# rusty-fast-solvers/rusty-compression

Hardware: AMD Instinct MI355X
Metric: GB/s + compressions/sec, 8192x8192 f64 rank-128 rSVD+ID (higher is better)
Workload: dtype f64

## Files before the change

### rusty_compression_amd/csrc/kernels_qr.hip

```cpp
#include "rc_common.hpp"
#include "rc_device.hpp"

namespace rc {

static __host__ __device__ inline int64_t cdiv(int64_t a, int64_t b) { return (a + b - 1) / b; }

template <typename T> struct Num;
template <> struct Num<double> {
    static __host__ __device__ inline double tol3z() { return 1.0536712127723509e-08; }
};
template <> struct Num<float> {
    static __host__ __device__ inline float tol3z() { return 2.44140625e-04f; }
};

template <typename T>
__device__ inline T wsum(T v) {
#pragma unroll
    for (int off = 32; off > 0; off >>= 1) v += __shfl_xor(v, off, 64);
    return v;
}

template <typename T, int TPC>
__device__ inline T group_sum(T v, T *sh ) {
    v = wsum(v);
    if (TPC == 256) {
        __syncthreads();
        if ((threadIdx.x & 63) == 0) sh[threadIdx.x >> 6] = v;
        __syncthreads();
        v = sh[0] + sh[1] + sh[2] + sh[3];
    }
    return v;
}

template <typename T>
// ... 239 lines not shown
    const int64_t m = w.rows, n = w.cols;
    if (m == 0 || n == 0) return;
    kmax = std::min(kmax, std::min(m, n));
    ProfScope ps(c, "op:geqp3 %lldx%lld k=%lld pivot=%d", (long long)m, (long long)n, (long long)kmax, pivot ? 1 : 0);
    T *vn1 = vn, *vn2 = vn + n;
    const int pv = pivot ? 1 : 0;
    hipLaunchKernelGGL(k_qr_init<T>, dim3((unsigned)std::min<int64_t>(n, 65535)), dim3(256), 0, c->stream, w, pv, jpvt, vn1, vn2);
    for (int64_t j = 0; j < kmax; ++j) {
        hipLaunchKernelGGL(k_qr_pivot_reflect<T>, dim3(1), dim3(1024), 0, c->stream, w, j, pv, jpvt, vn1, vn2, tau);
        const int64_t rem_cols = n - j - 1;
        if (rem_cols <= 0) continue;
        const int64_t rem = m - j;
        const int64_t c64 = cdiv(rem, 64), c256 = cdiv(rem, 256);
#define RC_APPLY(TPC, MAXE)                                                                                       \
    hipLaunchKernelGGL((k_qr_apply<T, TPC, MAXE>), dim3((unsigned)cdiv(rem_cols, 256 / TPC)), dim3(256), 0,      \
                       c->stream, w, j, pv, jpvt, vn1, vn2, tau)
        if (c64 <= 2 && rem_cols >= 2048) {
            constexpr int CPW = 4;
            hipLaunchKernelGGL((k_qr_apply_short<T, CPW>), dim3((unsigned)cdiv(rem_cols, 4 * CPW)), dim3(256), 0, c->stream, w, j, pv, jpvt, vn1, vn2, tau);
        }
        else if (c64 <= 2) RC_APPLY(64, 2);
        else if (c64 <= 8) RC_APPLY(64, 8);
        else if (c256 <= 8) RC_APPLY(256, 8);
        else if (c256 <= 16) RC_APPLY(256, 16);
        else if (c256 <= 32) RC_APPLY(256, 32);
        else
            hipLaunchKernelGGL(k_qr_apply_general<T>, dim3((unsigned)rem_cols), dim3(256), 0, c->stream, w, j, pv, jpvt, vn1, vn2, tau);
#undef RC_APPLY
    }
}

template <typename T>
__global__ __launch_bounds__(256) void k_extract_r(Mat<T> w, const int64_t *jpvt, Mat<T> r) {
    const bool col_fast = (r.cs <= r.rs);
    const int64_t total = r.rows * r.cols;
    for (int64_t e = blockIdx.x * (int64_t)blockDim.x + threadIdx.x; e < total; e += (int64_t)gridDim.x * blockDim.x) {
        int64_t i, p;
        if (col_fast) { i = e / r.cols; p = e - i * r.cols; }
        else { p = e / r.rows; i = e - p * r.rows; }
        r.at(i, p) = (i <= p) ? w.p[jpvt[p] * w.cs + i] : (T)0;
    }
}
template <typename T>
void extract_r(rc_context *c, Mat<T> w, const int64_t *jpvt, Mat<T> r) {
    if (r.empty()) return;
    int grid = (int)std::min<int64_t>(cdiv(r.rows * r.cols, 256), 8192);
    hipLaunchKernelGGL(k_extract_r<T>, dim3(grid), dim3(256), 0, c->stream, w, jpvt, r);
}

template <typename T, int MAXE>
__global__ __launch_bounds__(256) void k_form_q(Mat<T> w, const int64_t *jpvt, const T *tau, int64_t k, Mat<T> qw) {
    __shared__ T sh[4];
    const int64_t m = w.rows;
    const int64_t cq = blockIdx.x;
    const int tid = threadIdx.x;
    T x[MAXE];
#pragma unroll
    for (int e = 0; e < MAXE; ++e) {
        int64_t i = tid + (int64_t)e * 256;
        x[e] = (i == cq) ? (T)1 : (T)0;
    }
    for (int64_t j = (cq < k - 1 ? cq : k - 1); j >= 0; --j) {
        const T tj = tau[j];
        if (tj == (T)0) continue;
        const T *vcol = w.p + jpvt[j] * w.cs;
        T v[MAXE];
        T dot = 0;
#pragma unroll
        for (int e = 0; e < MAXE; ++e) {
            const int i = tid + e * 256;
            const bool ok = i < (int)m && i >= (int)j;
            const T vv = vcol[ok ? i : (int)j];
            v[e] = ok ? (i == (int)j ? (T)1 : vv) : (T)0;
            dot = fma(v[e], x[e], dot);
// ... 5 lines not shown
    }
    T *out = qw.p + cq * qw.cs;
#pragma unroll
    for (int e = 0; e < MAXE; ++e) {
        int64_t i = tid + (int64_t)e * 256;
        if (i < m) out[i] = x[e];
    }
}
template <typename T>
__global__ __launch_bounds__(256) void k_form_q_general(Mat<T> w, const int64_t *jpvt, const T *tau, int64_t k, Mat<T> qw) {
    __shared__ T sh[4];
    const int64_t m = w.rows;
    const int64_t cq = blockIdx.x;
    const int tid = threadIdx.x;
    T *x = qw.p + cq * qw.cs;
    for (int64_t i = tid; i < m; i += 256) x[i] = (i == cq) ? (T)1 : (T)0;
    for (int64_t j = (cq < k - 1 ? cq : k - 1); j >= 0; --j) {
        const T tj = tau[j];
        if (tj == (T)0) continue;
        const T *vcol = w.p + jpvt[j] * w.cs;
        const int64_t i0 = tid >= j ? tid : tid + ((j - tid + 255) / 256) * 256;
        T dot = 0;
        for (int64_t i = i0; i < m; i += 256) dot += ((i == j) ? (T)1 : vcol[i]) * x[i];
        dot = group_sum<T, 256>(dot, sh);
        const T f = tj * dot;
        for (int64_t i = i0; i < m; i += 256) x[i] -= f * ((i == j) ? (T)1 : vcol[i]);
    }
}

template <typename T, int NE>
__global__ __launch_bounds__(1024) void k_form_q_small(Mat<T> w, const int64_t *jpvt, const T *tau, int k, Mat<T> qw) {
    extern __shared__ __attribute__((aligned(16))) char smem_raw[];
    T *V = reinterpret_cast<T *>(smem_raw);
    T *tl = V + (size_t)k * 8 * NE;
    const int m = (int)w.rows;
    constexpr int LD = 8 * NE;
    for (int e = threadIdx.x; e < k * LD; e += blockDim.x) {
        const int j = e / LD, i = e - j * LD;
        V[e] = (i < j || i >= m) ? (T)0 : (i == j) ? (T)1 : w.p[jpvt[j] * w.cs + i];
    }
    for (int j = threadIdx.x; j < k; j += blockDim.x) tl[j] = tau[j];
    __syncthreads();
    const int l8 = threadIdx.x & 7, cq = threadIdx.x >> 3;
    if (cq >= qw.cols) return;
    T x[NE];
#pragma unroll
    for (int e = 0; e < NE; ++e) x[e] = (l8 + 8 * e == cq) ? (T)1 : (T)0;
    for (int j = cq < k - 1 ? cq : k - 1; j >= 0; --j) {
        const T tj = tl[j];
        if (tj == (T)0) continue;
        const T *vj = V + (size_t)j * LD + l8;
        T v[NE];
        T dot = 0;
#pragma unroll
        for (int e = 0; e < NE; ++e) {
            v[e] = vj[8 * e];
            dot = fma(v[e], x[e], dot);
        }
        dot = group_sum_dpp<8>(dot);
        const T f = tj * dot;
#pragma unroll
        for (int e = 0; e < NE; ++e) x[e] = fma(-f, v[e], x[e]);
    }
    T *out = qw.p + (int64_t)cq * qw.cs;
#pragma unroll
    for (int e = 0; e < NE; ++e) {
        const int i = l8 + 8 * e;
        if (i < m) out[i] = x[e];
    }
}

template <typename T>
__global__ __launch_bounds__(256) void k_extract_v(Mat<T> w, const int64_t *jpvt, Mat<T> vm) {
    const int64_t j = blockIdx.y;
    const T *col = w.p + jpvt[j] * w.cs;
    T *out = vm.p + j * vm.cs;
    for (int64_t i = blockIdx.x * 256 + threadIdx.x; i < vm.rows; i += (int64_t)gridDim.x * 256)
        out[i] = (i < j) ? (T)0 : (i == j) ? (T)1 : col[i];
}
template <typename T>
__global__ __launch_bounds__(1024) void k_build_t(Mat<T> sgram, const T *tau, Mat<T> tm) {
    extern __shared__ __attribute__((aligned(16))) char smem_raw[];
    T *svec = reinterpret_cast<T *>(smem_raw);
    T *trow = svec + tm.rows;
    const int k = (int)tm.rows;
    const int ld = k | 1;
    const int tid = threadIdx.x;
    for (int e = tid; e < k * ld; e += 1024) trow[e] = 0;
    __syncthreads();
    for (int j = 0; j < k; ++j) {
        for (int l = tid; l < j; l += 1024) svec[l] = sgram.at(l, j);
        __syncthreads();
        const T tj = tau[j];
        for (int i = tid; i <= j; i += 1024) {
            if (i == j) {
                trow[i * ld + j] = tj;
            } else {
                T acc = 0;
                for (int l = i; l < j; ++l) acc += trow[i * ld + l] * svec[l];
                trow[i * ld + j] = -tj * acc;
            }
        }
// ... 463 lines not shown
```

### rusty_compression_amd/csrc/kernels_wqcoop.hip

```cpp
#include "rc_common.hpp"
#include <cstdlib>
#include "rc_device.hpp"
#include "jacobi_lds.hpp"

#include <chrono>
#include <mutex>

#include <cerrno>
#include <csignal>
#include <fcntl.h>
#include <sys/file.h>
#include <sys/mman.h>
#include <unistd.h>

namespace rc {

namespace {

constexpr int kCoopMaxWgs = 128;
constexpr int kSpinLimit = 1 << 22;

template <typename T> struct Tol3z;
template <> struct Tol3z<double> { static __device__ inline double v() { return 1.0536712127723509e-08; } };
template <> struct Tol3z<float> { static __device__ inline float v() { return 2.44140625e-04f; } };

__device__ inline void st_agent(double *p, double v) { __hip_atomic_store(p, v, __ATOMIC_RELAXED, RC_AGENT); }
__device__ inline void st_agent(float *p, float v) { __hip_atomic_store(p, v, __ATOMIC_RELAXED, RC_AGENT); }
__device__ inline void st_agent(long long *p, long long v) { __hip_atomic_store(p, v, __ATOMIC_RELAXED, RC_AGENT); }
__device__ inline void st_agent(unsigned *p, unsigned v) { __hip_atomic_store(p, v, __ATOMIC_RELAXED, RC_AGENT); }
__device__ inline double ld_agent(const double *p) { return __hip_atomic_load(p, __ATOMIC_RELAXED, RC_AGENT); }
__device__ inline float ld_agent(const float *p) { return __hip_atomic_load(p, __ATOMIC_RELAXED, RC_AGENT); }
__device__ inline long long ld_agent(const long long *p) { return __hip_atomic_load(p, __ATOMIC_RELAXED, RC_AGENT); }
__device__ inline unsigned ld_agent(const unsigned *p) { return __hip_atomic_load(p, __ATOMIC_RELAXED, RC_AGENT); }

__global__ void k_coop_gate(unsigned *sem, unsigned need, unsigned budget, unsigned *sync, unsigned long long *hdr, int hdr_words, const int *proceed) {
    if (blockIdx.x != 0) return;
// ... 11 lines not shown
    }
    st_agent(sync + 1, ab);
}

}

#ifdef RC_COOP_TIMING
__device__ unsigned long long g_coop_dbg[8];
#endif

template <typename T>
struct WqCoopArgs {
    Mat<T> w;
    Mat<T> wf;
    int kmax;
    int cpw;
    int64_t *jpvt;
    T *tau;
    unsigned long long *hdr;
    T *cols;
    int mp;
    unsigned *sync;
    unsigned *sem;
    int *flag;
    int row0;
    int jend;
    const int *pos_in;
    int *pos_out;
    T *vn;
    unsigned units;
};

template <typename T, int NE, int CPG>
__device__ inline void wq_coop_body(const WqCoopArgs<T> &a, const int G, const int wg) {
    constexpr int NG = 64;
    constexpr int NW = 8;
    constexpr int kNoInt = 0x7fffffff;
    __shared__ double sh_v[NW];
    __shared__ int sh_p[NW], sh_c[NW], sh_j[NW];
    __shared__ int sh_exit;
    __shared__ int bc[4];
    __shared__ T xw[8 * NE];
    const int tid = threadIdx.x, lane = tid & 63, wv = tid >> 6, l8 = tid & 7, g8 = tid >> 3;
    const int m = (int)a.w.rows, mp = a.mp;
    const int64_t n = a.w.cols;
    const int c0 = wg * a.cpw;
    const int nloc = (int)((n - c0) < a.cpw ? (n - c0) : a.cpw);
    unsigned *done = a.sync, *abortw = a.sync + 1;

    const int row0 = a.row0;
    const unsigned ab0 = ld_agent(abortw);
    if (ab0 == 2u) {
        if (tid == 0 && wg == 0) atomicOr(a.flag, 4);
        return;
    }
    const bool dead = a.pos_in != nullptr && (__hip_atomic_load(a.flag, __ATOMIC_RELAXED, RC_AGENT) & 4) != 0;
    if (tid == 0) sh_exit = (ab0 != 0u) || dead;

    T x[CPG][NE];
    int pos[CPG];
    T myvn1 = 0, myvn2 = 0;
    const int mycol = c0 + g8 + NG * l8;
    const bool resumed = a.pos_in != nullptr;
    const Mat<T> src = resumed ? a.wf : a.w;
#pragma unroll
    for (int q = 0; q < CPG; ++q) {
        const int cl = g8 + NG * q;
        const bool valid = cl < nloc;
        const T *col = src.p + (int64_t)(c0 + (valid ? cl : 0)) * src.cs;
        const int64_t srs = src.rs;
        T ss = 0;
#pragma unroll
        for (int e = 0; e < NE; ++e) {
            const int i = row0 + l8 + 8 * e;
            x[q][e] = (valid && i < m) ? col[(int64_t)i * srs] : (T)0;
            ss = fma(x[q][e], x[q][e], ss);
        }
        ss = group_sum_dpp<8>(ss);
        if (l8 == q && !resumed) myvn1 = myvn2 = sqrt(ss);
        pos[q] = valid ? (resumed ? a.pos_in[c0 + cl] : c0 + cl) : -1;
    }
    if (resumed && l8 < CPG && g8 + NG * l8 < nloc) {
        myvn1 = a.vn[mycol];
        myvn2 = a.vn[n + mycol];
    }
    __syncthreads();
    bool aborted = sh_exit != 0;
// ... 220 lines not shown
    }
    rdone = r0 + 8;
    }
#undef RC_TICK
#ifdef RC_COOP_TIMING
    if (wg == 0 && tid == 0)
        for (int k2 = 0; k2 < 6; ++k2) g_coop_dbg[k2] = tph[k2];
#endif

    if (!aborted) {
#pragma unroll
        for (int q = 0; q < CPG; ++q) {
            if (pos[q] < 0) continue;
            T *col = a.wf.p + (int64_t)(c0 + g8 + NG * q) * a.wf.cs;
#pragma unroll
            for (int e = 0; e < NE; ++e) {
                const int i = rdone + l8 + 8 * e;
                if (i < m) col[i] = x[q][e];
            }
            if (l8 == 0) a.jpvt[pos[q]] = c0 + g8 + NG * q;
            if (l8 == 0 && a.pos_out) a.pos_out[c0 + g8 + NG * q] = pos[q];
        }
        if (a.pos_out && l8 < CPG && g8 + NG * l8 < nloc) {
            a.vn[mycol] = myvn1;
            a.vn[n + mycol] = myvn2;
        }
    }
    __syncthreads();
    if (tid == 0) {
        if (aborted && !dead) atomicOr(a.flag, 4);
        const unsigned old = __hip_atomic_fetch_add(done, 1u, __ATOMIC_ACQ_REL, RC_AGENT);
        if (old == (unsigned)G - 1u) __hip_atomic_fetch_sub(a.sem, a.units, __ATOMIC_RELAXED, RC_AGENT);
    }
}

template <typename T, int NE, int CPG>
__global__ __launch_bounds__(512, NE <= 4 ? 4 : 2) void k_wq_coop(WqCoopArgs<T> a) {
    wq_coop_body<T, NE, CPG>(a, (int)gridDim.x, (int)blockIdx.x);
}

template <typename T>
__global__ __launch_bounds__(512, 2) void k_wq_jacobi_fused(WqCoopArgs<T> a, JacobiLdsArgs<T> ja, int g) {
    const int wg = (int)blockIdx.x;
    if (wg < g) wq_coop_body<T, 16, 4>(a, g, wg);
    else jacobi_lds_body<T, 8, true, 2>(ja, wg == g + 1);
}

static unsigned *coop_semaphore(int device) {
    static std::mutex mu;
    static unsigned *sems[64] = {};
    std::lock_guard<std::mutex> lk(mu);
    unsigned *&s = sems[device & 63];
    if (!s) {
        RC_HIP(hipMalloc(reinterpret_cast<void **>(&s), 64));
        const unsigned zeros[16] = {};
        RC_HIP(hipMemcpy(s, zeros, 64, hipMemcpyHostToDevice));
    }
    return s;
}
void coop_prepare(int device) { (void)coop_semaphore(device); }
unsigned *coop_semaphore_of(int device) { return coop_semaphore(device); }

namespace {
struct ShareTable {
    uint32_t magic;
    uint32_t reserved;
    int32_t pids[62];
};
constexpr uint32_t kShareMagic = 0x52434350u;

struct DeviceShare {
    ShareTable *tab = nullptr;
    int fd = -1;
    bool tried = false;
    int live = 1;
    std::chrono::steady_clock::time_point stamp{};
};

// ... 129 lines not shown
        ProfScope ps(c, "op:geqp3_wide_coop %lldx%lld steps %lld..%lld wgs=%d", (long long)m, (long long)n, (long long)row0, (long long)jend, g);
        if (!last || !first) {
            if (!pos) {
                pos = c->alloc<int>((size_t)n);
                vn = c->alloc<T>((size_t)2 * n);
            }
        }
        WqCoopArgs<T> a = stage_args<T>(c, w, wf, kmax, jpvt, tau, flag, ne, g, cpw);
        a.row0 = (int)row0;
        a.jend = (int)jend;
        a.pos_in = first ? nullptr : pos;
        a.pos_out = last ? nullptr : pos;
        a.vn = vn;
        coop_gate_launch(c, a.units, a.sync, a.hdr, 2 * g * 5);
#define RC_COOP(NE_, CPG_) hipLaunchKernelGGL((k_wq_coop<T, NE_, CPG_>), dim3((unsigned)g), dim3(512), 0, c->stream, a)
        if (ne == 4) RC_COOP(4, 8);
        else if (ne == 8) RC_COOP(8, 8);
        else if (ne == 16) RC_COOP(16, 4);
        else RC_COOP(32, 2);
#undef RC_COOP
        row0 = jend;
        first = false;
    }
}

template <typename T>
bool wide_coop_jacobi_supported(int64_t m, int64_t n, int device) {
    if (!std::is_same<T, double>::value) return false;
    return m == 8 * kLPP && stage_ne(m) == 16 && wide_coop_supported<T>(m, n, device) &&
           jacobi_lds_bytes<T>((int)m, jacobi_pitch<T>((int)m)) <= kJacobiLdsCap;
}

template <typename T>
void geqp3_wide_coop_jacobi(rc_context *c, Mat<T> w, Mat<T> wf, int64_t kmax, int64_t *jpvt, T *tau, int *flag, Mat<T> core, Mat<T> uc, T *s, Mat<T> vc) {
    const int64_t m = w.rows, n = w.cols;
    RC_REQUIRE(wf.rs == 1 && wf.rows == m && wf.cols == n, RC_LAYOUT_ERROR, "geqp3_wide_coop_jacobi: column-major output required");
    RC_REQUIRE(core.rows == m && core.cols == m && core.rs == 1 && uc.rs == 1 && vc.rs == 1, RC_LAYOUT_ERROR, "geqp3_wide_coop_jacobi: square column-major core required");
    RC_REQUIRE(wide_coop_jacobi_supported<T>(m, n, c->device), RC_INVALID_ARGUMENT, "geqp3_wide_coop_jacobi: unsupported shape");
    if constexpr (std::is_same<T, double>::value) {
        kmax = std::min(kmax, std::min(m, n));
        const int nc = (int)m, N = nc;
        int cpg, cpw, g;
        stage_shape(16, n, &cpg, &cpw, &g);
        ProfScope ps(c, "op:geqp3_wide_coop %lldx%lld + jacobi_svd n=%d wgs=%d+2", (long long)m, (long long)n, nc, g);
        const WqCoopArgs<T> a = stage_args<T>(c, w, wf, kmax, jpvt, tau, flag, 16, g, cpw);
        const int ld = jacobi_pitch<T>(nc);
        const size_t lds = jacobi_lds_bytes<T>(nc, ld);
        const size_t nrec = (size_t)kMaxSweeps * (N - 1) * (N / 2);
        Rot<T> *log = c->alloc<Rot<T>>(nrec);
        int *sweeps = c->alloc<int>(1);
        int *order = c->alloc<int>((size_t)nc);
        unsigned *vsync = c->alloc<unsigned>((size_t)nc + 1);
        unsigned long long *chk = c->alloc<unsigned long long>(nrec);
        const JacobiLdsArgs<T> ja{core, log, sweeps, uc, s, order, kMaxSweeps, 1, vsync, chk, c->epoch_word(), vc, c->health_word(), ld};
        auto kern = k_wq_jacobi_fused<T>;
        static bool attr_set[64] = {};
        if (!attr_set[c->device & 63]) {
            RC_HIP(hipFuncSetAttribute(reinterpret_cast<const void *>(kern), hipFuncAttributeMaxDynamicSharedMemorySize, 160 * 1024 - 2048));
            attr_set[c->device & 63] = true;
        }
        fill_words(c, vsync, ((size_t)nc + 1) * sizeof(unsigned), 0u);
        coop_gate_launch(c, a.units, a.sync, a.hdr, 2 * g * 5);
        hipLaunchKernelGGL(kern, dim3((unsigned)g + 2), dim3(512), lds, c->stream, a, ja, g);
    }
}

#ifdef RC_COOP_TIMING
extern "C" void rc_debug_coop_timing(unsigned long long *out) { (void)hipMemcpyFromSymbol(out, HIP_SYMBOL(g_coop_dbg), 8 * sizeof(unsigned long long)); }
#endif
template bool wide_coop_supported<double>(int64_t, int64_t, int);
template bool wide_coop_supported<float>(int64_t, int64_t, int);
template void geqp3_wide_coop<double>(rc_context *, Mat<double>, Mat<double>, int64_t, int64_t *, double *, int *);
template void geqp3_wide_coop<float>(rc_context *, Mat<float>, Mat<float>, int64_t, int64_t *, float *, int *);
template bool wide_coop_jacobi_supported<double>(int64_t, int64_t, int);
template bool wide_coop_jacobi_supported<float>(int64_t, int64_t, int);
template void geqp3_wide_coop_jacobi<double>(rc_context *, Mat<double>, Mat<double>, int64_t, int64_t *, double *, int *, Mat<double>, Mat<double>, double *, Mat<double>);
template void geqp3_wide_coop_jacobi<float>(rc_context *, Mat<float>, Mat<float>, int64_t, int64_t *, float *, int *, Mat<float>, Mat<float>, float *, Mat<float>);

}
```

### rusty_compression_amd/csrc/rc_api.hip

```cpp
#include "rc_common.hpp"

#include <unistd.h>

#include <atomic>
#include <chrono>

#include <algorithm>
#include <cmath>

using namespace rc;

static constexpr size_t kAlign = 256;

void rc_context::retire_arena() {
    if (arena) {
        if (live_graphs > 0) retired.push_back(arena);
        else (void)hipFree(arena);
    }
    arena = nullptr;
    arena_size = 0;
}

void rc_context::swap_arena() {
    std::swap(arena, aux_arena.base);
// ... 418 lines not shown
            done = run_certified(c, [&](int *flag) { tsqr_cholqr2<T>(c, wt, qw, transposed ? core.t() : core, flag); });
        }
    }
    const bool factored = done && fold;
    if (!done) {
        qw = tmp_colmajor<T>(c, M, r);
        int64_t *jp = c->alloc<int64_t>((size_t)std::max<int64_t>(r, 1));
        T *tau = c->alloc<T>((size_t)std::max<int64_t>(r, 1));
        T *vn = c->alloc<T>((size_t)std::max<int64_t>(2 * r, 1));
        geqp3_inplace(c, wt, r, false, jp, tau, vn);
        extract_r(c, wt, jp, transposed ? core.t() : core);
        form_q(c, wt, jp, tau, r, qw);
    }
    Mat<T> vwork = tmp_colmajor<T>(c, r, r), uc = tmp_colmajor<T>(c, r, r), vc = tmp_colmajor<T>(c, r, r);
    jacobi_svd(c, core, vwork, uc, s, vc);
    svd_finish(c, transposed, factored, qw, q1, r2i, uc, vc, s, u, vt);
}

template <typename T>
void compute_svd(rc_context *c, Mat<T> a, Mat<T> u, T *s, Mat<T> vt) {
    const int64_t m = a.rows, n = a.cols, r = std::min(m, n);
    RC_REQUIRE(u.rows == m && u.cols == r && vt.rows == r && vt.cols == n, RC_INVALID_ARGUMENT,
               "compute_svd: a %lld x %lld needs u %lld x %lld, vt %lld x %lld", (long long)m, (long long)n, (long long)m,
               (long long)r, (long long)r, (long long)n);
    if (r == 0) return;
    ArenaMark mark(c);
    const bool transposed = m < n;
    Mat<T> src = transposed ? a.t() : a;
    Mat<T> wt = tmp_colmajor<T>(c, src.rows, src.cols);
    copy_mat(c, src, wt);
    svd_core(c, wt, transposed, u, s, vt);
}

template <typename T>
void qr_column_id(rc_context *c, Mat<T> q, Mat<T> r, const int64_t *ind, Mat<T> cm, Mat<T> z) {
    const int64_t m = q.rows, k = q.cols, n = r.cols;
    RC_REQUIRE(r.rows == k && cm.rows == m && cm.cols == k && z.rows == k && z.cols == n, RC_INVALID_ARGUMENT,
               "column_id: q %lld x %lld, r %lld x %lld, c %lld x %lld, z %lld x %lld", (long long)m, (long long)k,
               (long long)r.rows, (long long)n, (long long)cm.rows, (long long)cm.cols, (long long)z.rows, (long long)z.cols);
    RC_REQUIRE(k <= n, RC_INVALID_ARGUMENT, "column_id: rank exceeds the number of columns");
    if (n == 0) return;
    ArenaMark mark(c);
    static const int fused = [] { const char *e = getenv("RC_ID_FUSED"); return e ? atoi(e) : 1; }();
    if (fused && k < n) {
        id_z_from_r(c, r, k, ind, z);
        gemm<T>(c, 1, q, r.sub(0, k, 0, k), 0, cm);
        return;
    }
    int64_t *inv = c->alloc<int64_t>((size_t)n);
    invert_perm(c, ind, n, inv);
    Mat<T> zt = tmp_rowmajor<T>(c, k, n);
    if (k == n) {
        gemm<T>(c, 1, q, r, 0, cm);
        fill_identity(c, zt);
    } else {
        fill_identity(c, zt.sub(0, k, 0, k));
        copy_mat(c, r.sub(0, k, k, n - k), zt.sub(0, k, k, n - k));
        trsm_upper(c, r.sub(0, k, 0, k), zt.sub(0, k, k, n - k));
        gemm<T>(c, 1, q, r.sub(0, k, 0, k), 0, cm);
    }
    gather_cols(c, zt, inv, z);
}

template <typename T>
void lq_row_id(rc_context *c, Mat<T> l, Mat<T> q, const int64_t *ind, Mat<T> x, Mat<T> rrows) {
    qr_column_id(c, q.t(), l.t(), ind, rrows.t(), x.t());
}

template <typename T>
void project_dense(rc_context *c, Mat<T> range, Mat<T> a, Mat<T> b) {
    gemm<T>(c, 1, range.t(), a, 0, b);
}

template <typename T>
struct OpView {
    int64_t rows = 0, cols = 0;
    Mat<T> dense;
    const rc_operator *cb = nullptr;
// ... 251 lines not shown
    }
    Mat<T> b = tmp_rowmajor<T>(c, k, n);
    {
        ProfScope ps(c, "stage:project B=Q^H A");
        a.project(c, range, b);
    }
    rsvd_id_consumers(c, range, b, o);
}

template <typename T>
bool fused_consumers_qualify(rc_context *c, int64_t k, int64_t n) {
    return c->opt_fused_consumers && c->opt_wide_coop && c->opt_tsqr && tsqr_fold() && c->lanes_in_flight() < 8 && tsqr_supported<T>(n, k) &&
           wide_coop_jacobi_supported<T>(k, n, c->device);
}

template <typename T>
bool rsvd_id_consumers_fused(rc_context *c, Mat<T> range, Mat<T> b, const rc_rsvd_id_out &o) {
    const int64_t m = range.rows, k = b.rows, n = b.cols;
    ArenaMark mark(c);
    Mat<T> core = tmp_colmajor<T>(c, k, k);
    Mat<T> q1 = rowmajor(c->alloc<T>((size_t)n * even_ld(k)), n, k, even_ld(k));
    Mat<T> r2i = rowmajor(c->alloc<T>((size_t)k * even_ld(k)), k, k, even_ld(k));
    {
        ProfScope ps(c, "stage:tall QR of B^T");
        if (!run_certified(c, [&](int *flag) { tsqr_cholqr2_factored<T>(c, b.t(), q1, r2i, core.t(), flag); })) return false;
    }
    Mat<T> uc = tmp_colmajor<T>(c, k, k), vc = tmp_colmajor<T>(c, k, k);
    Mat<T> qb = tmp_colmajor<T>(c, k, k);
    Mat<T> r = o.qr_r.data ? from_c<T>(o.qr_r) : tmp_rowmajor<T>(c, k, n);
    int64_t *ind = o.qr_ind ? o.qr_ind : c->alloc<int64_t>((size_t)n);
    T *tau = c->alloc<T>((size_t)k);
    Mat<T> wf = tmp_colmajor<T>(c, k, n);
    T *s = static_cast<T *>(o.s);
    bool qr_done;
    {
        ProfScope ps(c, "stage:qrcp of B | svd of the core");
        qr_done = run_certified(c, [&](int *flag) { geqp3_wide_coop_jacobi<T>(c, b, wf, k, ind, tau, flag, core, uc, s, vc); });
    }
    {
        ProfScope ps(c, "stage:qrcp of B + column_id");
        if (qr_done) {
            extract_r(c, wf, ind, r);
            form_q(c, wf, ind, tau, k, qb);
        } else {
            qrcp_core(c, b, k, true, qb, r, ind);
        }
        Mat<T> q = o.qr_q.data ? from_c<T>(o.qr_q) : tmp_colmajor<T>(c, m, k);
        gemm<T>(c, 1, range, qb, 0, q);
        if (o.id_c.data || o.id_z.data) qr_column_id(c, q, r, ind, from_c<T>(o.id_c), from_c<T>(o.id_z));
    }
    {
        ProfScope ps(c, "stage:svd of B + U=Q Ub");
        Mat<T> ub = tmp_colmajor<T>(c, k, k);
        svd_finish(c, true, true, Mat<T>(), q1, r2i, uc, vc, s, ub, from_c<T>(o.vt));
        gemm<T>(c, 1, range, ub, 0, from_c<T>(o.u));
    }
    return true;
}

template <typename T>
void rsvd_id_consumers(rc_context *c, Mat<T> range, Mat<T> b, const rc_rsvd_id_out &o) {
    const int64_t m = range.rows, k = b.rows, n = b.cols;
    const bool want_id = o.id_c.data || o.id_z.data || o.qr_q.data || o.qr_r.data || o.qr_ind;
    const bool want_svd = o.u.data || o.s || o.vt.data;
    if (want_svd) RC_REQUIRE(o.u.data && o.s && o.vt.data, RC_INVALID_ARGUMENT, "rsvd_id: u, s, vt must be given together");
    if (want_id && want_svd && !c->opt_fork && fused_consumers_qualify<T>(c, k, n)) {
        RC_REQUIRE(!(o.id_c.data || o.id_z.data) || (o.id_c.data && o.id_z.data), RC_INVALID_ARGUMENT, "rsvd_id: id_c and id_z must be given together");
        if (rsvd_id_consumers_fused(c, range, b, o)) return;
    }
    Mat<T> wq;
    if (want_id && want_svd && c->opt_fork) {
        wq = tmp_colmajor<T>(c, k, n);
        copy_mat(c, b, wq);
    }
    Fork fork(c, want_svd && want_id);
    if (want_id) {
        ProfScope ps(c, "stage:qrcp of B + column_id");
        Mat<T> qb = tmp_colmajor<T>(c, k, k);
        Mat<T> r = o.qr_r.data ? from_c<T>(o.qr_r) : tmp_rowmajor<T>(c, k, n);
        int64_t *ind = o.qr_ind ? o.qr_ind : c->alloc<int64_t>((size_t)n);
        if (wq.p) qrcp_core(c, wq, k, true, qb, r, ind);
        else qrcp_core(c, b, k, true, qb, r, ind, want_svd);
// ... 392 lines not shown
}
rc_status rc_graph_launch(rc_context *ctx, void *graph_exec) {
    if (!ctx || !graph_exec) return RC_INVALID_ARGUMENT;
    DeviceGuard dg(ctx->device);
    hipError_t e = hipGraphLaunch(static_cast<hipGraphExec_t>(graph_exec), ctx->stream);
    if (e != hipSuccess) { ctx->last_error = hipGetErrorString(e); return RC_RUNTIME_ERROR; }
    return RC_OK;
}
rc_status rc_graph_destroy(rc_context *ctx, void *graph_exec) {
    if (!ctx) return RC_INVALID_ARGUMENT;
    if (!graph_exec) return RC_OK;
    DeviceGuard dg(ctx->device);
    (void)hipStreamSynchronize(ctx->stream);
    (void)hipGraphExecDestroy(static_cast<hipGraphExec_t>(graph_exec));
    if (ctx->live_graphs > 0 && --ctx->live_graphs == 0) {
        for (void *p : ctx->retired) (void)hipFree(p);
        ctx->retired.clear();
    }
    return RC_OK;
}

rc_status rc_set_option(rc_context *ctx, int32_t option, int64_t value) {
    if (!ctx) return RC_INVALID_ARGUMENT;
    switch (option) {
        case RC_OPT_TALL_SKINNY_FAST_PATH: ctx->opt_tsqr = value != 0; return RC_OK;
        case RC_OPT_WIDE_LAZY_QRCP: ctx->opt_wide_lazy = value != 0; return RC_OK;
        case RC_OPT_WIDE_COOP_QRCP: ctx->opt_wide_coop = value != 0; return RC_OK;
        case RC_OPT_POWER_ITERATION_FIXED: ctx->opt_power_fixed = value != 0; return RC_OK;
        case RC_OPT_FORK_BRANCHES: ctx->opt_fork = value != 0; return RC_OK;
        case RC_OPT_BLOCKED_QRCP: ctx->opt_blocked = value != 0; return RC_OK;
        case RC_OPT_COOP_PANEL: ctx->opt_coop_panel = value != 0; return RC_OK;
        case RC_OPT_CONCURRENCY_HINT: ctx->opt_lanes = (int)std::max<int64_t>(1, std::min<int64_t>(value, 1024)); return RC_OK;
        case RC_OPT_KERNEL_SLOTS: ctx->opt_slots = (int)std::max<int64_t>(1, std::min<int64_t>(value, 1024)); return RC_OK;
        case RC_OPT_FUSED_CONSUMERS: ctx->opt_fused_consumers = value != 0; return RC_OK;
        default: ctx->last_error = "unknown option"; return RC_INVALID_ARGUMENT;
    }
}
rc_status rc_get_health(rc_context *ctx, int32_t *word) {
    if (!ctx || !word) return RC_INVALID_ARGUMENT;
    DeviceGuard dg(ctx->device);
    *word = 0;
    if (!ctx->health) return RC_OK;
    int h = 0;
    if (debug_memset_path() & 2) {
        hipError_t e = hipStreamSynchronize(ctx->stream);
        if (e == hipSuccess) e = hipMemcpy(&h, ctx->health, sizeof(int), hipMemcpyDeviceToHost);
        if (e == hipSuccess) e = hipMemset(ctx->health, 0, sizeof(int));
        if (e != hipSuccess) { ctx->last_error = hipGetErrorString(e); return RC_RUNTIME_ERROR; }
        *word = h;
        return RC_OK;
    }
    try {
        read_back(ctx, ctx->health, &h, 1);
        hipLaunchKernelGGL(k_set_word, dim3(1), dim3(64), 0, ctx->stream, ctx->health, 0);
        RC_HIP(hipStreamSynchronize(ctx->stream));
    } catch (const Error &e) { ctx->last_error = e.msg; return e.code; }
    *word = h;
    return RC_OK;
}

rc_status rc_profile_enable(rc_context *ctx, int32_t on) {
    if (!ctx) return RC_INVALID_ARGUMENT;
    ctx->prof_on = on != 0;
    return RC_OK;
}
rc_status rc_profile_reset(rc_context *ctx) {
    if (!ctx) return RC_INVALID_ARGUMENT;
// ... 275 lines not shown
```

### rusty_compression_amd/csrc/rc_common.hpp

```cpp
#pragma once

#include <hip/hip_runtime.h>

#include <cstdarg>
#include <cstdint>
#include <cstdio>
#include <cstring>
#include <map>
#include <string>
#include <vector>

#include "../../include/rusty_compression_amd.h"

namespace rc {

template <typename T>
struct Mat {
    T *p = nullptr;
    int64_t rows = 0, cols = 0, rs = 0, cs = 0;

    __host__ __device__ Mat() {}
    __host__ __device__ Mat(T *p_, int64_t r, int64_t c, int64_t rs_, int64_t cs_) : p(p_), rows(r), cols(c), rs(rs_), cs(cs_) {}
    __host__ __device__ inline T &at(int64_t i, int64_t j) const { return p[i * rs + j * cs]; }
    __host__ __device__ Mat<T> sub(int64_t r0, int64_t nr, int64_t c0, int64_t nc) const {
// ... 44 lines not shown
struct rc_context {
    int device = 0;
    hipStream_t stream = nullptr;
    std::string last_error;
    std::string last_gemm_kernel;

    int call_depth = 0;
    char *arena = nullptr;
    size_t arena_size = 0;
    size_t arena_off = 0;
    size_t arena_high = 0;
    std::vector<void *> overflow;
    int live_graphs = 0;
    std::vector<void *> retired;
    void retire_arena();
    hipStream_t aux_stream = nullptr;
    hipEvent_t fork_ev = nullptr, join_ev = nullptr;
    struct ArenaState { char *base = nullptr; size_t size = 0, off = 0, high = 0; std::vector<void *> overflow; } aux_arena;
    void swap_arena();
    int opt_fork = 0;
    hipEvent_t sync_ev = nullptr;
    void *pinned = nullptr;
    size_t pinned_size = 0;
    int pinned_cursor = 0;

    int opt_tsqr = 1;
    int opt_power_fixed = 0;
    int opt_wide_coop = 1;
    int opt_wide_lazy = 1;
    int opt_blocked = 1;
    int opt_coop_panel = 1;
    int opt_lanes = 1;
    int opt_slots = 4;
    int opt_fused_consumers = 1;
    int lanes_in_flight() const { return opt_lanes < opt_slots ? opt_lanes : opt_slots; }
    int *health = nullptr;
    int *health_word();
    unsigned *epoch = nullptr;
    unsigned *epoch_word();

    bool capturing = false;
    bool prof_on = false;
    struct ProfPending { std::string name; hipEvent_t beg, end; };
    struct ProfAcc { double ms = 0; int64_t calls = 0; };
    std::vector<ProfPending> prof_pending;
    std::vector<hipEvent_t> prof_free;
    std::map<std::string, ProfAcc> prof_acc;
    hipEvent_t prof_event();
    void prof_resolve();

    void reset_arena();
    void *alloc_bytes(size_t bytes);
    template <typename T>
    T *alloc(size_t n) { return static_cast<T *>(alloc_bytes(n * sizeof(T))); }
    void reserve(size_t bytes);
    void release_all();
};

namespace rc {

struct ProfScope {
    rc_context *c;
    hipEvent_t beg = nullptr;
    std::string name;
    ProfScope(rc_context *ctx, const char *fmt, ...) : c(ctx) {
        if (!c->prof_on || c->capturing) return;
        char buf[160];
// ... 53 lines not shown
void invert_perm(rc_context *c, const int64_t *perm, int64_t n, int64_t *inv);
void fill_words(rc_context *c, void *p, size_t bytes, unsigned v);
void iota_i64(rc_context *c, int64_t *p, int64_t n);
template <typename T> void col_sumsq(rc_context *c, Mat<T> a, T *out);
template <typename T> void max_sqrt(rc_context *c, const T *v, int64_t n, T *out);
template <typename T> void fro_diff(rc_context *c, Mat<T> a, Mat<T> b, T *out2);
template <typename T> void adaptive_residual_update(rc_context *c, Mat<T> y, Mat<T> corr);

template <typename T> void gemm(rc_context *c, T alpha, Mat<T> a, Mat<T> b, T beta, Mat<T> cmat);
template <typename T> void complete_left_basis(rc_context *c, Mat<T> uc, const T *s);

template <typename T> void geqp3_inplace(rc_context *c, Mat<T> w, int64_t kmax, bool pivot, int64_t *jpvt, T *tau, T *vn);
template <typename T> bool geqp3_blocked_supported(int64_t m, int64_t n, int64_t kmax);
template <typename T> void geqp3_blocked(rc_context *c, Mat<T> w, int64_t kmax, int64_t *jpvt, T *tau, Mat<T> q_out, Mat<T> restore_from = Mat<T>());
template <typename T> struct BlockedQrcpJob;
template <typename T> BlockedQrcpJob<T> *qrb_begin(rc_context *c, Mat<T> w, int64_t kmax, int64_t *jpvt, T *tau);
template <typename T> void qrb_issue(BlockedQrcpJob<T> *job);
template <typename T> bool qrb_finish(BlockedQrcpJob<T> *job);
template <typename T> void qrb_form_q(BlockedQrcpJob<T> *job, Mat<T> q);
template <typename T> void qrb_end(BlockedQrcpJob<T> *job);
struct QrbState;
template <typename T> bool qrb_optimistic_possible(BlockedQrcpJob<T> *job);
template <typename T> bool qrb_issue_all_optimistic(BlockedQrcpJob<T> *job);
template <typename T> bool qrb_verify_optimistic(BlockedQrcpJob<T> *job);
template <typename T> bool qrb_verify_optimistic(const QrbState *host_log, const std::vector<int> &nbp_log, bool broken);
template <typename T> void qrb_optimistic_log(BlockedQrcpJob<T> *job, const QrbState **log, std::vector<int> *nbp_log, bool *broken);
template <typename T> void qrb_keep_t(BlockedQrcpJob<T> *job, bool keep);
template <typename T> bool wide_lazy_supported(int64_t m, int64_t n);
template <typename T> void geqp3_wide_lazy(rc_context *c, Mat<T> b, int64_t kmax, int64_t *jpvt, Mat<T> q, Mat<T> r);
template <typename T> bool wide_coop_supported(int64_t m, int64_t n, int device);
template <typename T> void geqp3_wide_coop(rc_context *c, Mat<T> w, Mat<T> wf, int64_t kmax, int64_t *jpvt, T *tau, int *flag);
template <typename T> bool wide_coop_jacobi_supported(int64_t m, int64_t n, int device);
template <typename T>
void geqp3_wide_coop_jacobi(rc_context *c, Mat<T> w, Mat<T> wf, int64_t kmax, int64_t *jpvt, T *tau, int *flag, Mat<T> core, Mat<T> uc, T *s, Mat<T> vc);
void coop_prepare(int device);
unsigned *coop_semaphore_of(int device);
unsigned coop_budget_units(int device);
void coop_gate_launch(rc_context *c, unsigned need, unsigned *sync, unsigned long long *hdr, int hdr_words, const int *proceed = nullptr);
template <typename T> void extract_r(rc_context *c, Mat<T> w, const int64_t *jpvt, Mat<T> r);
template <typename T> void form_q(rc_context *c, Mat<T> w, const int64_t *jpvt, const T *tau, int64_t k, Mat<T> qw);
template <typename T> void trsm_upper(rc_context *c, Mat<T> t, Mat<T> b);
template <typename T> bool tsqr_supported(int64_t m, int64_t n);
template <typename T> void tsqr_cholqr2(rc_context *c, Mat<T> y, Mat<T> q, Mat<T> r, int *flag);
template <typename T> void tsqr_cholqr2_factored(rc_context *c, Mat<T> y, Mat<T> q1, Mat<T> r2i, Mat<T> r, int *flag);
template <typename T> void qrcp_small(rc_context *c, Mat<T> rin, int64_t kmax, bool pivot, int64_t *jpvt, Mat<T> rout, Mat<T> q2);
template <typename T> void householder_sign_fix(rc_context *c, Mat<T> q, Mat<T> r);
template <typename T> void qrcp_tall_fast(rc_context *c, Mat<T> y, int64_t k, bool pivot, Mat<T> q, Mat<T> r, int64_t *ind, int *flag);
template <typename T> void jacobi_svd(rc_context *c, Mat<T> g, Mat<T> vwork, Mat<T> uc, T *s, Mat<T> vc);

}
```

Before: 658.0.

## Fuse R extraction, Q formation and ID Z solve into cooperative QRCP kernel tail

```diff
diff --git a/rusty_compression_amd/csrc/kernels_qr.hip b/rusty_compression_amd/csrc/kernels_qr.hip
--- a/rusty_compression_amd/csrc/kernels_qr.hip
+++ b/rusty_compression_amd/csrc/kernels_qr.hip
@@ -1,5 +1,6 @@
 #include "rc_common.hpp"
 #include "rc_device.hpp"
+#include "qr_tail.hpp"
 
 namespace rc {
 
@@ -305,14 +306,7 @@
 
 template <typename T>
 __global__ __launch_bounds__(256) void k_extract_r(Mat<T> w, const int64_t *jpvt, Mat<T> r) {
-    const bool col_fast = (r.cs <= r.rs);
-    const int64_t total = r.rows * r.cols;
-    for (int64_t e = blockIdx.x * (int64_t)blockDim.x + threadIdx.x; e < total; e += (int64_t)gridDim.x * blockDim.x) {
-        int64_t i, p;
-        if (col_fast) { i = e / r.cols; p = e - i * r.cols; }
-        else { p = e / r.rows; i = e - p * r.rows; }
-        r.at(i, p) = (i <= p) ? w.p[jpvt[p] * w.cs + i] : (T)0;
-    }
+    extract_r_body<T>(w, jpvt, r, threadIdx.x, blockDim.x, blockIdx.x, gridDim.x);
 }
 template <typename T>
 void extract_r(rc_context *c, Mat<T> w, const int64_t *jpvt, Mat<T> r) {
@@ -384,42 +378,10 @@
 __global__ __launch_bounds__(1024) void k_form_q_small(Mat<T> w, const int64_t *jpvt, const T *tau, int k, Mat<T> qw) {
     extern __shared__ __attribute__((aligned(16))) char smem_raw[];
     T *V = reinterpret_cast<T *>(smem_raw);
-    T *tl = V + (size_t)k * 8 * NE;
-    const int m = (int)w.rows;
-    constexpr int LD = 8 * NE;
-    for (int e = threadIdx.x; e < k * LD; e += blockDim.x) {
-        const int j = e / LD, i = e - j * LD;
-        V[e] = (i < j || i >= m) ? (T)0 : (i == j) ? (T)1 : w.p[jpvt[j] * w.cs + i];
-    }
-    for (int j = threadIdx.x; j < k; j += blockDim.x) tl[j] = tau[j];
-    __syncthreads();
+    form_q_small_stage<T, NE>(w, jpvt, tau, k, V, threadIdx.x, blockDim.x);
     const int l8 = threadIdx.x & 7, cq = threadIdx.x >> 3;
     if (cq >= qw.cols) return;
-    T x[NE];
-#pragma unroll
-    for (int e = 0; e < NE; ++e) x[e] = (l8 + 8 * e == cq) ? (T)1 : (T)0;
-    for (int j = cq < k - 1 ? cq : k - 1; j >= 0; --j) {
-        const T tj = tl[j];
-        if (tj == (T)0) continue;
-        const T *vj = V + (size_t)j * LD + l8;
-        T v[NE];
-        T dot = 0;
-#pragma unroll
-        for (int e = 0; e < NE; ++e) {
-            v[e] = vj[8 * e];
-            dot = fma(v[e], x[e], dot);
-        }
-        dot = group_sum_dpp<8>(dot);
-        const T f = tj * dot;
-#pragma unroll
-        for (int e = 0; e < NE; ++e) x[e] = fma(-f, v[e], x[e]);
-    }
-    T *out = qw.p + (int64_t)cq * qw.cs;
-#pragma unroll
-    for (int e = 0; e < NE; ++e) {
-        const int i = l8 + 8 * e;
-        if (i < m) out[i] = x[e];
-    }
+    form_q_small_column<T, NE>(w, k, qw, V, cq, l8);
 }
 
 template <typename T>
diff --git a/rusty_compression_amd/csrc/kernels_wqcoop.hip b/rusty_compression_amd/csrc/kernels_wqcoop.hip
--- a/rusty_compression_amd/csrc/kernels_wqcoop.hip
+++ b/rusty_compression_amd/csrc/kernels_wqcoop.hip
@@ -2,6 +2,7 @@
 #include <cstdlib>
 #include "rc_device.hpp"
 #include "jacobi_lds.hpp"
+#include "qr_tail.hpp"
 
 #include <chrono>
 #include <mutex>
@@ -79,7 +80,7 @@
 };
 
 template <typename T, int NE, int CPG>
-__device__ inline void wq_coop_body(const WqCoopArgs<T> &a, const int G, const int wg) {
+__device__ inline bool wq_coop_body(const WqCoopArgs<T> &a, const int G, const int wg) {
     constexpr int NG = 64;
     constexpr int NW = 8;
     constexpr int kNoInt = 0x7fffffff;
@@ -99,7 +100,7 @@
     const unsigned ab0 = ld_agent(abortw);
     if (ab0 == 2u) {
         if (tid == 0 && wg == 0) atomicOr(a.flag, 4);
-        return;
+        return false;
     }
     const bool dead = a.pos_in != nullptr && (__hip_atomic_load(a.flag, __ATOMIC_RELAXED, RC_AGENT) & 4) != 0;
     if (tid == 0) sh_exit = (ab0 != 0u) || dead;
@@ -386,18 +387,68 @@
         const unsigned old = __hip_atomic_fetch_add(done, 1u, __ATOMIC_ACQ_REL, RC_AGENT);
         if (old == (unsigned)G - 1u) __hip_atomic_fetch_sub(a.sem, a.units, __ATOMIC_RELAXED, RC_AGENT);
     }
+    return !aborted;
 }
 
 template <typename T, int NE, int CPG>
 __global__ __launch_bounds__(512, NE <= 4 ? 4 : 2) void k_wq_coop(WqCoopArgs<T> a) {
-    wq_coop_body<T, NE, CPG>(a, (int)gridDim.x, (int)blockIdx.x);
+    (void)wq_coop_body<T, NE, CPG>(a, (int)gridDim.x, (int)blockIdx.x);
 }
 
 template <typename T>
-__global__ __launch_bounds__(512, 2) void k_wq_jacobi_fused(WqCoopArgs<T> a, JacobiLdsArgs<T> ja, int g) {
+__device__ inline void wq_tail(const WqCoopArgs<T> &a, const WqTailArgs<T> &t, const int G, const int wg, const bool finished) {
+    __shared__ int sh_go;
+    extern __shared__ __attribute__((aligned(16))) char smem_raw[];
+    const int tid = threadIdx.x;
+    unsigned *arrived = a.sync + 2, *abortw = a.sync + 1;
+    asm volatile("s_waitcnt vmcnt(0)" ::: "memory");
+    __syncthreads();
+    if (tid == 0) {
+        bool go = false;
+        if (finished) {
+            __builtin_amdgcn_fence(__ATOMIC_RELEASE, "agent");
+            asm volatile("s_waitcnt vmcnt(0)" ::: "memory");
+            __hip_atomic_fetch_add(arrived, 1u, __ATOMIC_RELAXED, RC_AGENT);
+            for (int it = 0; it <= kSpinLimit; ++it) {
+                if (ld_agent(arrived) == (unsigned)G) { go = true; break; }
+                if ((it & 31) == 31 && ld_agent(abortw) != 0u) break;
+                __builtin_amdgcn_s_sleep(1);
+            }
+            if (go) {
+                __builtin_amdgcn_fence(__ATOMIC_ACQUIRE, "agent");
+            } else {
+                st_agent(abortw, 1u);
+                atomicOr(a.flag, 4);
+            }
+        }
+        sh_go = go ? 1 : 0;
+    }
+    asm volatile("s_waitcnt vmcnt(0)" ::: "memory");
+    __syncthreads();
+    if (!sh_go) return;
+    const int64_t k = a.kmax;
+    if (t.z.p) {
+        const int64_t nb = (a.wf.cols + 255) / 256;
+        for (int64_t blk = wg; blk < nb; blk += G) id_z_body<T, false, true>(a.wf, a.jpvt, k, t.z, (unsigned)tid, 256u, (unsigned)blk);
+    }
+    if (t.r.p) extract_r_body<T>(a.wf, a.jpvt, t.r, (unsigned)tid, 512u, (unsigned)wg, (unsigned)G);
+    if (t.qb.p && wg == G - 1) {
+        T *V = reinterpret_cast<T *>(smem_raw);
+        __syncthreads();
+        form_q_small_stage<T, 16>(a.wf, a.jpvt, a.tau, (int)k, V, (unsigned)tid, 512u);
+        for (int cq = tid >> 3; cq < (int)t.qb.cols; cq += 64) form_q_small_column<T, 16>(a.wf, (int)k, t.qb, V, cq, tid & 7);
+    }
+}
+
+template <typename T, bool TAIL>
+__global__ __launch_bounds__(512, 2) void k_wq_jacobi_fused(WqCoopArgs<T> a, JacobiLdsArgs<T> ja, int g, WqTailArgs<T> ta) {
     const int wg = (int)blockIdx.x;
-    if (wg < g) wq_coop_body<T, 16, 4>(a, g, wg);
-    else jacobi_lds_body<T, 8, true, 2>(ja, wg == g + 1);
+    if (wg < g) {
+        const bool finished = wq_coop_body<T, 16, 4>(a, g, wg);
+        if constexpr (TAIL) wq_tail<T>(a, ta, g, wg, finished);
+    } else {
+        jacobi_lds_body<T, 8, true, 2>(ja, wg == g + 1);
+    }
 }
 
 static unsigned *coop_semaphore(int device) {
@@ -593,7 +644,8 @@
 }
 
 template <typename T>
-void geqp3_wide_coop_jacobi(rc_context *c, Mat<T> w, Mat<T> wf, int64_t kmax, int64_t *jpvt, T *tau, int *flag, Mat<T> core, Mat<T> uc, T *s, Mat<T> vc) {
+void geqp3_wide_coop_jacobi(rc_context *c, Mat<T> w, Mat<T> wf, int64_t kmax, int64_t *jpvt, T *tau, int *flag, Mat<T> core, Mat<T> uc, T *s, Mat<T> vc,
+                            const WqTailArgs<T> *tail) {
     const int64_t m = w.rows, n = w.cols;
     RC_REQUIRE(wf.rs == 1 && wf.rows == m && wf.cols == n, RC_LAYOUT_ERROR, "geqp3_wide_coop_jacobi: column-major output required");
     RC_REQUIRE(core.rows == m && core.cols == m && core.rs == 1 && uc.rs == 1 && vc.rs == 1, RC_LAYOUT_ERROR, "geqp3_wide_coop_jacobi: square column-major core required");
@@ -614,15 +666,27 @@
         unsigned *vsync = c->alloc<unsigned>((size_t)nc + 1);
         unsigned long long *chk = c->alloc<unsigned long long>(nrec);
         const JacobiLdsArgs<T> ja{core, log, sweeps, uc, s, order, kMaxSweeps, 1, vsync, chk, c->epoch_word(), vc, c->health_word(), ld};
-        auto kern = k_wq_jacobi_fused<T>;
-        static bool attr_set[64] = {};
-        if (!attr_set[c->device & 63]) {
-            RC_HIP(hipFuncSetAttribute(reinterpret_cast<const void *>(kern), hipFuncAttributeMaxDynamicSharedMemorySize, 160 * 1024 - 2048));
-            attr_set[c->device & 63] = true;
+        WqTailArgs<T> ta;
+        if (tail) {
+            ta = *tail;
+            RC_REQUIRE(kmax == m, RC_INVALID_ARGUMENT, "geqp3_wide_coop_jacobi: the tail needs all %lld steps", (long long)m);
+            RC_REQUIRE(!ta.r.p || (ta.r.rows == m && ta.r.cols == n), RC_INVALID_ARGUMENT, "geqp3_wide_coop_jacobi: tail r must be %lld x %lld", (long long)m, (long long)n);
+            RC_REQUIRE(!ta.qb.p || (ta.qb.rows == m && ta.qb.cols == m && ta.qb.rs == 1), RC_LAYOUT_ERROR, "geqp3_wide_coop_jacobi: tail qb must be column-major %lld x %lld", (long long)m, (long long)m);
+            RC_REQUIRE(!ta.z.p || (ta.z.rows == m && ta.z.cols == n && m < n), RC_INVALID_ARGUMENT, "geqp3_wide_coop_jacobi: tail z must be %lld x %lld", (long long)m, (long long)n);
+        }
+        const size_t lds_tail = tail && ta.qb.p ? ((size_t)kmax * 8 * 16 + (size_t)kmax) * sizeof(T) : 0;
+        const size_t lds_launch = std::max(lds, lds_tail);
+        const size_t lds_cap = 160 * 1024 - (tail ? 4096 : 2048);
+        RC_REQUIRE(lds_launch <= lds_cap, RC_INVALID_ARGUMENT, "geqp3_wide_coop_jacobi: %zu bytes of LDS", lds_launch);
+        auto kern = tail ? k_wq_jacobi_fused<T, true> : k_wq_jacobi_fused<T, false>;
+        static bool attr_set[64][2] = {};
+        if (!attr_set[c->device & 63][tail ? 1 : 0]) {
+            RC_HIP(hipFuncSetAttribute(reinterpret_cast<const void *>(kern), hipFuncAttributeMaxDynamicSharedMemorySize, (int)lds_cap));
+            attr_set[c->device & 63][tail ? 1 : 0] = true;
         }
         fill_words(c, vsync, ((size_t)nc + 1) * sizeof(unsigned), 0u);
         coop_gate_launch(c, a.units, a.sync, a.hdr, 2 * g * 5);
-        hipLaunchKernelGGL(kern, dim3((unsigned)g + 2), dim3(512), lds, c->stream, a, ja, g);
+        hipLaunchKernelGGL(kern, dim3((unsigned)g + 2), dim3(512), lds_launch, c->stream, a, ja, g, ta);
     }
 }
 
@@ -635,7 +699,7 @@
 template void geqp3_wide_coop<float>(rc_context *, Mat<float>, Mat<float>, int64_t, int64_t *, float *, int *);
 template bool wide_coop_jacobi_supported<double>(int64_t, int64_t, int);
 template bool wide_coop_jacobi_supported<float>(int64_t, int64_t, int);
-template void geqp3_wide_coop_jacobi<double>(rc_context *, Mat<double>, Mat<double>, int64_t, int64_t *, double *, int *, Mat<double>, Mat<double>, double *, Mat<double>);
-template void geqp3_wide_coop_jacobi<float>(rc_context *, Mat<float>, Mat<float>, int64_t, int64_t *, float *, int *, Mat<float>, Mat<float>, float *, Mat<float>);
-
-}
+template void geqp3_wide_coop_jacobi<double>(rc_context *, Mat<double>, Mat<double>, int64_t, int64_t *, double *, int *, Mat<double>, Mat<double>, double *, Mat<double>, const WqTailArgs<double> *);
+template void geqp3_wide_coop_jacobi<float>(rc_context *, Mat<float>, Mat<float>, int64_t, int64_t *, float *, int *, Mat<float>, Mat<float>, float *, Mat<float>, const WqTailArgs<float> *);
+
+}
diff --git a/rusty_compression_amd/csrc/qr_tail.hpp b/rusty_compression_amd/csrc/qr_tail.hpp
--- /dev/null
+++ b/rusty_compression_amd/csrc/qr_tail.hpp
@@ -0,0 +1,119 @@
+#pragma once
+#include "rc_common.hpp"
+#include "rc_device.hpp"
+
+namespace rc {
+
+template <typename T>
+__device__ inline void extract_r_body(const Mat<T> &w, const int64_t *jpvt, const Mat<T> &r, const unsigned tid, const unsigned nt, const unsigned blk, const unsigned nblk) {
+    const bool col_fast = (r.cs <= r.rs);
+    const int64_t total = r.rows * r.cols;
+    for (int64_t e = blk * (int64_t)nt + tid; e < total; e += (int64_t)nblk * nt) {
+        int64_t i, p;
+        if (col_fast) { i = e / r.cols; p = e - i * r.cols; }
+        else { p = e / r.rows; i = e - p * r.rows; }
+        r.at(i, p) = (i <= p) ? w.p[jpvt[p] * w.cs + i] : (T)0;
+    }
+}
+
+template <typename T, int NE>
+__device__ inline void form_q_small_stage(const Mat<T> &w, const int64_t *jpvt, const T *tau, const int k, T *V, const unsigned tid, const unsigned nt) {
+    T *tl = V + (size_t)k * 8 * NE;
+    const int m = (int)w.rows;
+    constexpr int LD = 8 * NE;
+    for (int e = tid; e < k * LD; e += nt) {
+        const int j = e / LD, i = e - j * LD;
+        V[e] = (i < j || i >= m) ? (T)0 : (i == j) ? (T)1 : w.p[jpvt[j] * w.cs + i];
+    }
+    for (int j = tid; j < k; j += nt) tl[j] = tau[j];
+    __syncthreads();
+}
+template <typename T, int NE>
+__device__ inline void form_q_small_column(const Mat<T> &w, const int k, const Mat<T> &qw, const T *V, const int cq, const int l8) {
+    const T *tl = V + (size_t)k * 8 * NE;
+    const int m = (int)w.rows;
+    constexpr int LD = 8 * NE;
+    T x[NE];
+#pragma unroll
+    for (int e = 0; e < NE; ++e) x[e] = (l8 + 8 * e == cq) ? (T)1 : (T)0;
+    for (int j = cq < k - 1 ? cq : k - 1; j >= 0; --j) {
+        const T tj = tl[j];
+        if (tj == (T)0) continue;
+        const T *vj = V + (size_t)j * LD + l8;
+        T v[NE];
+        T dot = 0;
+#pragma unroll
+        for (int e = 0; e < NE; ++e) {
+            v[e] = vj[8 * e];
+            dot = fma(v[e], x[e], dot);
+        }
+        dot = group_sum_dpp<8>(dot);
+        const T f = tj * dot;
+#pragma unroll
+        for (int e = 0; e < NE; ++e) x[e] = fma(-f, v[e], x[e]);
+    }
+    T *out = qw.p + (int64_t)cq * qw.cs;
+#pragma unroll
+    for (int e = 0; e < NE; ++e) {
+        const int i = l8 + 8 * e;
+        if (i < m) out[i] = x[e];
+    }
+}
+
+template <typename T, bool FROM_R, bool WIDE>
+__device__ inline void id_z_body(const Mat<T> &w, const int64_t *jpvt, const int64_t k, const Mat<T> &z, const unsigned tid, const unsigned nt, const unsigned blk) {
+    constexpr int NB = 16;
+    __shared__ T tile[NB][NB + 1];
+    const bool worker = !WIDE || tid < nt;
+    const int64_t n = w.cols;
+    const int64_t p = blk * (int64_t)nt + tid;
+    const bool inside = worker && p < n;
+    const int64_t dc = inside ? jpvt[p] : 0;
+    const bool active = inside && p >= k;
+    const T *bcol = FROM_R ? w.p + (inside ? p : 0) * w.cs : w.p + dc * w.cs;
+    const int64_t brs = FROM_R ? w.rs : 1;
+    const int64_t nblk = (k + NB - 1) / NB;
+    const int ti = tid / NB, tj = tid % NB;
+    if (inside && p < k)
+        for (int64_t i = 0; i < k; ++i) z.at(i, dc) = (i == p) ? (T)1 : (T)0;
+    for (int64_t bi = nblk - 1; bi >= 0; --bi) {
+        const int64_t r0 = bi * NB;
+        T acc[NB];
+#pragma unroll
+        for (int ii = 0; ii < NB; ++ii) acc[ii] = (active && r0 + ii < k) ? bcol[(r0 + ii) * brs] : (T)0;
+        for (int64_t bj = nblk - 1; bj >= bi; --bj) {
+            const int64_t c0 = bj * NB;
+            __syncthreads();
+            if (worker) {
+                const int64_t i = r0 + ti, l = c0 + tj;
+                tile[ti][tj] = (i < k && l < k && i <= l) ? (FROM_R ? w.at(i, l) : w.p[jpvt[l] * w.cs + i]) : (T)0;
+            }
+            __syncthreads();
+            if (bj > bi) {
+                T x[NB];
+#pragma unroll
+                for (int jj = 0; jj < NB; ++jj) x[jj] = (active && c0 + jj < k) ? z.at(c0 + jj, dc) : (T)0;
+#pragma unroll
+                for (int jj = 0; jj < NB; ++jj)
+#pragma unroll
+                    for (int ii = 0; ii < NB; ++ii) acc[ii] -= tile[ii][jj] * x[jj];
+            } else {
+#pragma unroll
+                for (int ii = NB - 1; ii >= 0; --ii) {
+                    if (r0 + ii < k) {
+                        acc[ii] /= tile[ii][ii];
+#pragma unroll
+                        for (int i2 = 0; i2 < ii; ++i2) acc[i2] -= tile[i2][ii] * acc[ii];
+                    }
+                }
+            }
+        }
+        if (active) {
+#pragma unroll
+            for (int ii = 0; ii < NB; ++ii)
+                if (r0 + ii < k) z.at(r0 + ii, dc) = acc[ii];
+        }
+    }
+}
+
+}
diff --git a/rusty_compression_amd/csrc/rc_api.hip b/rusty_compression_amd/csrc/rc_api.hip
--- a/rusty_compression_amd/csrc/rc_api.hip
+++ b/rusty_compression_amd/csrc/rc_api.hip
@@ -474,8 +474,13 @@
     svd_core(c, wt, transposed, u, s, vt);
 }
 
-template <typename T>
-void qr_column_id(rc_context *c, Mat<T> q, Mat<T> r, const int64_t *ind, Mat<T> cm, Mat<T> z) {
+static bool id_z_one_launch() {
+    static const int fused = [] { const char *e = getenv("RC_ID_FUSED"); return e ? atoi(e) : 1; }();
+    return fused != 0;
+}
+
+template <typename T>
+void qr_column_id(rc_context *c, Mat<T> q, Mat<T> r, const int64_t *ind, Mat<T> cm, Mat<T> z, bool z_done = false) {
     const int64_t m = q.rows, k = q.cols, n = r.cols;
     RC_REQUIRE(r.rows == k && cm.rows == m && cm.cols == k && z.rows == k && z.cols == n, RC_INVALID_ARGUMENT,
                "column_id: q %lld x %lld, r %lld x %lld, c %lld x %lld, z %lld x %lld", (long long)m, (long long)k,
@@ -483,9 +488,9 @@
     RC_REQUIRE(k <= n, RC_INVALID_ARGUMENT, "column_id: rank exceeds the number of columns");
     if (n == 0) return;
     ArenaMark mark(c);
-    static const int fused = [] { const char *e = getenv("RC_ID_FUSED"); return e ? atoi(e) : 1; }();
-    if (fused && k < n) {
-        id_z_from_r(c, r, k, ind, z);
+    RC_REQUIRE(!z_done || (id_z_one_launch() && k < n), RC_INVALID_ARGUMENT, "column_id: Z cannot be in place on this path");
+    if (id_z_one_launch() && k < n) {
+        if (!z_done) id_z_from_r(c, r, k, ind, z);
         gemm<T>(c, 1, q, r.sub(0, k, 0, k), 0, cm);
         return;
     }
@@ -803,22 +808,30 @@
     T *tau = c->alloc<T>((size_t)k);
     Mat<T> wf = tmp_colmajor<T>(c, k, n);
     T *s = static_cast<T *>(o.s);
+    const bool in_tail = c->opt_fused_consumers >= 2;
+    const bool z_in_tail = in_tail && o.id_z.data && id_z_one_launch() && k < n;
+    WqTailArgs<T> tail;
     bool qr_done;
     {
         ProfScope ps(c, "stage:qrcp of B | svd of the core");
-        qr_done = run_certified(c, [&](int *flag) { geqp3_wide_coop_jacobi<T>(c, b, wf, k, ind, tau, flag, core, uc, s, vc); });
+        if (in_tail) {
+            tail.r = r;
+            tail.qb = qb;
+            if (z_in_tail) tail.z = from_c<T>(o.id_z);
+        }
+        qr_done = run_certified(c, [&](int *flag) { geqp3_wide_coop_jacobi<T>(c, b, wf, k, ind, tau, flag, core, uc, s, vc, in_tail ? &tail : nullptr); });
     }
     {
         ProfScope ps(c, "stage:qrcp of B + column_id");
-        if (qr_done) {
+        if (qr_done && !in_tail) {
             extract_r(c, wf, ind, r);
             form_q(c, wf, ind, tau, k, qb);
-        } else {
+        } else if (!qr_done) {
             qrcp_core(c, b, k, true, qb, r, ind);
         }
         Mat<T> q = o.qr_q.data ? from_c<T>(o.qr_q) : tmp_colmajor<T>(c, m, k);
         gemm<T>(c, 1, range, qb, 0, q);
-        if (o.id_c.data || o.id_z.data) qr_column_id(c, q, r, ind, from_c<T>(o.id_c), from_c<T>(o.id_z));
+        if (o.id_c.data || o.id_z.data) qr_column_id(c, q, r, ind, from_c<T>(o.id_c), from_c<T>(o.id_z), qr_done && z_in_tail);
     }
     {
         ProfScope ps(c, "stage:svd of B + U=Q Ub");
@@ -1277,7 +1290,7 @@
         case RC_OPT_COOP_PANEL: ctx->opt_coop_panel = value != 0; return RC_OK;
         case RC_OPT_CONCURRENCY_HINT: ctx->opt_lanes = (int)std::max<int64_t>(1, std::min<int64_t>(value, 1024)); return RC_OK;
         case RC_OPT_KERNEL_SLOTS: ctx->opt_slots = (int)std::max<int64_t>(1, std::min<int64_t>(value, 1024)); return RC_OK;
-        case RC_OPT_FUSED_CONSUMERS: ctx->opt_fused_consumers = value != 0; return RC_OK;
+        case RC_OPT_FUSED_CONSUMERS: ctx->opt_fused_consumers = value <= 0 ? 0 : value >= 2 ? 2 : 1; return RC_OK;
         default: ctx->last_error = "unknown option"; return RC_INVALID_ARGUMENT;
     }
 }
diff --git a/rusty_compression_amd/csrc/rc_common.hpp b/rusty_compression_amd/csrc/rc_common.hpp
--- a/rusty_compression_amd/csrc/rc_common.hpp
+++ b/rusty_compression_amd/csrc/rc_common.hpp
@@ -100,7 +100,7 @@
     int opt_coop_panel = 1;
     int opt_lanes = 1;
     int opt_slots = 4;
-    int opt_fused_consumers = 1;
+    int opt_fused_consumers = 2;
     int lanes_in_flight() const { return opt_lanes < opt_slots ? opt_lanes : opt_slots; }
     int *health = nullptr;
     int *health_word();
@@ -220,7 +220,12 @@
 template <typename T> void geqp3_wide_coop(rc_context *c, Mat<T> w, Mat<T> wf, int64_t kmax, int64_t *jpvt, T *tau, int *flag);
 template <typename T> bool wide_coop_jacobi_supported(int64_t m, int64_t n, int device);
 template <typename T>
-void geqp3_wide_coop_jacobi(rc_context *c, Mat<T> w, Mat<T> wf, int64_t kmax, int64_t *jpvt, T *tau, int *flag, Mat<T> core, Mat<T> uc, T *s, Mat<T> vc);
+struct WqTailArgs {
+    Mat<T> r, qb, z;
+};
+template <typename T>
+void geqp3_wide_coop_jacobi(rc_context *c, Mat<T> w, Mat<T> wf, int64_t kmax, int64_t *jpvt, T *tau, int *flag, Mat<T> core, Mat<T> uc, T *s, Mat<T> vc,
+                            const WqTailArgs<T> *tail = nullptr);
 void coop_prepare(int device);
 unsigned *coop_semaphore_of(int device);
 unsigned coop_budget_units(int device);
```

Result: faster. 675.1 (median of 6 runs) (+2.6%).
